# upowai/upow

Measured on AMD Instinct MI355X. Metric: sha256_pow_hashrate_MH/s, higher is better.
Workload: dtype uint32; 1 GPU; model=upow v2 block header PoW (108 B, single SHA-256, nibble-prefix target), global_batch=4294967296, seq_len=108, parallelism=dp1, nonces_per_rank_step=4294967296, device=gpu, kernel_variant=0

## Files before the change

### csrc/bindings.cpp

```cpp
#include <pybind11/numpy.h>
#include <pybind11/pybind11.h>
#include <pybind11/stl.h>

#include <cstring>
#include <malloc.h>
#include <stdexcept>

#include "native.h"
#include "sha256_common.h"
#include "thread_pool.h"

namespace py = pybind11;
using namespace upow;

namespace upow {
void register_txcodec(py::module_& m);
void register_ledger_writer(py::module_& m);
void register_gov_index(py::module_& m);
void register_stall_probe(py::module_& m);
void register_log_appender(py::module_& m);
void register_http_wire(py::module_& m);
void register_mempool_index(py::module_& m);
void register_jsonspan(py::module_& m);
void register_utxo_host(py::module_& m);
}

static PowJobHost make_job(py::bytes header, uint32_t tmask, uint32_t tword, uint32_t frac_shift,
                           uint32_t frac_limit) {
    PowJobHost j;
    std::string h = header;
    j.header.assign(h.begin(), h.end());
    j.tmask = tmask;
    j.tword = tword;
    j.frac_shift = frac_shift;
    j.frac_limit = frac_limit;
    return j;
}

static py::tuple pow_result_tuple(const PowResult& r) {
    return py::make_tuple(r.searched, r.total_hits, r.words);
}

static void packed_args(py::buffer data, py::buffer offsets, const uint8_t*& d, const int64_t*& o, int64_t& n,
                        int64_t& nbytes) {
    py::buffer_info di = data.request(), oi = offsets.request();
    if (oi.itemsize != 8 || oi.ndim != 1) throw std::invalid_argument("offsets must be a 1-D int64 buffer");
    d = static_cast<const uint8_t*>(di.ptr);
    o = static_cast<const int64_t*>(oi.ptr);
    n = oi.shape[0] - 1;
    nbytes = di.size * di.itemsize;
    if (n < 0) throw std::invalid_argument("offsets must have n+1 entries");
    for (int64_t i = 0; i < n; ++i)
        if (o[i] < 0 || o[i + 1] < o[i] || o[i + 1] > nbytes) throw std::out_of_range("bad offsets");
}

PYBIND11_MODULE(_native, m) {
    m.doc() = "upow_amd native core: host C++ crypto + gfx950 HIP kernels";
    register_txcodec(m);
    register_ledger_writer(m);
    register_gov_index(m);
    register_stall_probe(m);
    register_log_appender(m);
    register_http_wire(m);
    register_mempool_index(m);
    register_jsonspan(m);
    register_utxo_host(m);

    m.def("malloc_tune", [](int64_t mmap_threshold, int64_t trim_threshold) {
        bool ok = true;
        if (mmap_threshold > 0) ok &= mallopt(M_MMAP_THRESHOLD, int(std::min<int64_t>(mmap_threshold, INT32_MAX))) == 1;
        if (trim_threshold > 0) ok &= mallopt(M_TRIM_THRESHOLD, int(std::min<int64_t>(trim_threshold, INT32_MAX))) == 1;
        return ok;
    });

    m.def("sha256", [](py::bytes msg) {
        std::string s = msg;
        uint8_t out[32];
        host_sha256(reinterpret_cast<const uint8_t*>(s.data()), s.size(), out);
        return py::bytes(reinterpret_cast<const char*>(out), 32);
    });

    m.def("sha256_batch_host", [](py::buffer data, py::buffer offsets, int threads) {
        const uint8_t* d; const int64_t* o; int64_t n, nb;
        packed_args(data, offsets, d, o, n, nb);
        std::vector<uint8_t> out;
        {
            py::gil_scoped_release rel;
            out = sha256_batch_host(d, o, n, threads);
        }
        return py::bytes(reinterpret_cast<const char*>(out.data()), out.size());
    }, py::arg("data"), py::arg("offsets"), py::arg("threads") = 1);

    m.def("sha256_hex_prefixes", [](py::list hexes, py::array_t<int64_t, py::array::c_style | py::array::forcecast> idx,
                                   py::array_t<int64_t, py::array::c_style | py::array::forcecast> nchars, int threads) {
        const int64_t n = int64_t(idx.size());
        if (int64_t(nchars.size()) != n) throw py::value_error("sha256_hex_prefixes: idx and nchars differ in length");
        const int64_t* ix = idx.data();
        const int64_t* nc = nchars.data();
        std::vector<const char*> src(static_cast<size_t>(n));
        std::vector<py::object> keep;
        keep.reserve(static_cast<size_t>(n));
        const int64_t n_hex = int64_t(hexes.size());
        for (int64_t k = 0; k < n; ++k) {
            if (ix[k] < 0 || ix[k] >= n_hex) throw py::index_error("sha256_hex_prefixes: tx index out of range");
            PyObject* o = PyList_GET_ITEM(hexes.ptr(), Py_ssize_t(ix[k]));
            keep.push_back(py::reinterpret_borrow<py::object>(o));
            if (!PyUnicode_Check(o)) throw py::type_error("transaction hex must be str");
            Py_ssize_t sz = 0;
            const char* p = PyUnicode_AsUTF8AndSize(o, &sz);
            if (!p) throw py::error_already_set();
            if (nc[k] < 0 || nc[k] > int64_t(sz)) throw py::value_error("sha256_hex_prefixes: prefix longer than the hex");
            src[size_t(k)] = p;
        }
        std::string out(size_t(n) * 32, '\0');
        {
            py::gil_scoped_release rel;
            HostPool::get().parallel_for(n, threads, [&](int64_t k) {
                host_sha256(reinterpret_cast<const uint8_t*>(src[size_t(k)]), size_t(nc[k]),
                            reinterpret_cast<uint8_t*>(&out[size_t(k) * 32]));
            });
        }
        return py::bytes(out);
    }, py::arg("hexes"), py::arg("idx"), py::arg("nchars"), py::arg("threads") = 1);

    m.def("sha256_batch_gpu", [](py::buffer data, py::buffer offsets) {
        const uint8_t* d; const int64_t* o; int64_t n, nb;
        packed_args(data, offsets, d, o, n, nb);
        std::vector<uint8_t> out;
        {
            py::gil_scoped_release rel;
            out = sha256_batch_gpu(d, nb, o, n);
        }
        return py::bytes(reinterpret_cast<const char*>(out.data()), out.size());
    });

    m.def("pow_check_word", [](py::bytes header, uint32_t tmask, uint32_t tword, uint32_t fs, uint32_t fl,
                               uint32_t v) { return pow_check_word_host(make_job(header, tmask, tword, fs, fl), v); });

    m.def("pow_variant_count", []() { return pow_variant_count(); });
    m.def("pow_job_h0", [](py::bytes header, uint32_t v) { return pow_job_h0_host(make_job(header, 0, 0, 0, 16), v); },
          py::arg("header"), py::arg("v"),
          "digest word H0 for nonce word v, from the precomputed job constants of the GPU kernel (host arithmetic)");

    m.def("pow_search_host", [](py::bytes header, uint32_t tmask, uint32_t tword, uint32_t fs, uint32_t fl,
                                uint64_t start, uint64_t count, int threads) {
        PowJobHost j = make_job(header, tmask, tword, fs, fl);
        PowResult r;
        {
            py::gil_scoped_release rel;
            r = pow_search_host(j, start, count, threads);
        }
        return pow_result_tuple(r);
    });

    m.def("pow_search_gpu", [](py::bytes header, uint32_t tmask, uint32_t tword, uint32_t fs, uint32_t fl,
                               uint64_t start, uint64_t count, int grid_blocks, uint32_t chunk_iters, uint32_t cap, int variant) {
        PowJobHost j = make_job(header, tmask, tword, fs, fl);
        PowResult r;
        {
            py::gil_scoped_release rel;
            r = pow_search_gpu(j, start, count, grid_blocks, chunk_iters, cap, variant);
        }
        return pow_result_tuple(r);
    }, py::arg("header"), py::arg("tmask"), py::arg("tword"), py::arg("frac_shift"), py::arg("frac_limit"),
       py::arg("start"), py::arg("count"), py::arg("grid_blocks") = 0, py::arg("chunk_iters") = 0,
       py::arg("cap") = 1 << 16, py::arg("variant") = 0);

    m.def("set_node_device", [](int dev) { set_node_device_native(dev); }, py::arg("device"),
          "pin node-side GPU work (verify, decompress, batched SHA-256) to this device from every thread");
    m.def("pow_kernel_info", [](int variant) {
        PowKernelInfo k = pow_kernel_info(variant);
        return py::dict(py::arg("cus") = k.cus, py::arg("blocks_per_cu") = k.blocks_per_cu,
                        py::arg("resident_blocks") = k.resident_blocks);
    }, py::arg("variant") = 0);
    m.def("p256_verify", [](py::buffer items, bool gpu, int threads) {
        py::buffer_info bi = items.request();
        const int64_t nbytes = bi.size * bi.itemsize;
        if (nbytes % 160) throw std::invalid_argument("items must be n x 160 bytes");
        const int64_t n = nbytes / 160;
        const uint8_t* p = static_cast<const uint8_t*>(bi.ptr);
        std::vector<uint8_t> st;
        {
            py::gil_scoped_release rel;
            st = gpu ? p256_verify_gpu(p, n) : p256_verify_host(p, n, threads);
        }
        return py::bytes(reinterpret_cast<const char*>(st.data()), st.size());
    }, py::arg("items"), py::arg("gpu") = false, py::arg("threads") = 1);

    m.def("p256_decompress", [](py::buffer in, bool gpu) {
        py::buffer_info bi = in.request();
        const int64_t nbytes = bi.size * bi.itemsize;
        if (nbytes % 33) throw std::invalid_argument("input must be n x 33 bytes");
        const int64_t n = nbytes / 33;
        std::vector<uint8_t> out(static_cast<size_t>(n) * 64), ok(static_cast<size_t>(n));
        {
            py::gil_scoped_release rel;
            if (gpu) p256_decompress_gpu(static_cast<const uint8_t*>(bi.ptr), n, out.data(), ok.data());
            else p256_decompress_host(static_cast<const uint8_t*>(bi.ptr), n, out.data(), ok.data());
        }
        return py::make_tuple(py::bytes(reinterpret_cast<const char*>(out.data()), out.size()),
                              py::bytes(reinterpret_cast<const char*>(ok.data()), ok.size()));
    }, py::arg("data"), py::arg("gpu") = false);

    m.def("p256_on_curve", [](py::buffer in, bool gpu, int threads) {
        py::buffer_info bi = in.request();
        const int64_t nbytes = bi.size * bi.itemsize;
        if (nbytes % 64) throw std::invalid_argument("input must be n x 64 bytes (x LE | y LE)");
        const int64_t n = nbytes / 64;
        std::string ok(static_cast<size_t>(n), '\0');
        {
            py::gil_scoped_release rel;
            auto* o = reinterpret_cast<uint8_t*>(&ok[0]);
            if (gpu) p256_on_curve_gpu(static_cast<const uint8_t*>(bi.ptr), n, o);
            else p256_on_curve_host(static_cast<const uint8_t*>(bi.ptr), n, o, threads);
        }
        return py::bytes(ok);
    }, py::arg("data"), py::arg("gpu") = false, py::arg("threads") = 8);

    m.def("p256_pubkey", [](py::bytes d_be) -> py::object {
        std::string d = d_be;
        if (d.size() != 32) throw std::invalid_argument("private key must be 32 bytes big-endian");
        uint8_t out[64];
        if (!p256_pubkey(reinterpret_cast<const uint8_t*>(d.data()), out)) return py::none();
        return py::bytes(reinterpret_cast<const char*>(out), 64);
    });

    m.def("p256_scalar_inv_mont", [](py::bytes s_le) -> py::bytes {
        const std::string s = s_le;
        if (s.size() != 32) throw std::invalid_argument("need 32 bytes little-endian");
        uint64_t in[4], out[4];
        std::memcpy(in, s.data(), 32);
        p256_scalar_inv_mont_host(out, in);
        return py::bytes(reinterpret_cast<const char*>(out), 32);
    });

    m.def("p256_fe_ops", [](py::bytes a_le, py::bytes b_le) -> py::bytes {
        const std::string a = a_le, b = b_le;
        if (a.size() != 32 || b.size() != 32) throw std::invalid_argument("need 32-byte little-endian a, b");
        uint32_t x[8], y[8], out[32];
        std::memcpy(x, a.data(), 32);
        std::memcpy(y, b.data(), 32);
        p256_fe_ops_host(x, y, out);
        return py::bytes(reinterpret_cast<const char*>(out), sizeof out);
    });
    m.def("rccl_unique_id", []() { return py::bytes(rccl_unique_id()); });
    m.def("rccl_vote_create", [](py::bytes uid, int world, int rank) {
        const std::string u = uid;
        py::gil_scoped_release rel;
        return rccl_vote_create(u, world, rank);
    });
    m.def("rccl_vote_start", [](int64_t h, int value) { rccl_vote_start(h, value); });
    m.def("rccl_vote_finish", [](int64_t h, double timeout_s) {
        py::gil_scoped_release rel;
        return rccl_vote_finish(h, timeout_s);
    });
    m.def("rccl_vote_stats", [](int64_t h) { return rccl_vote_stats(h); });
    m.def("rccl_vote_destroy", [](int64_t h, bool abort) {
        py::gil_scoped_release rel;
        rccl_vote_destroy(h, abort);
    }, py::arg("h"), py::arg("abort") = false);
    m.def("p256_g16_entries", [](int64_t first, int64_t count) -> py::bytes {
        std::vector<uint8_t> o;
        { py::gil_scoped_release rel; o = p256_g16_entries(first, count); }
        return py::bytes(reinterpret_cast<const char*>(o.data()), o.size());
    });
    m.def("p256_fe_reduce", [](py::bytes c_le) -> py::bytes {
        const std::string c = c_le;
        if (c.size() != 64) throw std::invalid_argument("need 64 bytes little-endian");
        uint32_t x[16], out[8];
        std::memcpy(x, c.data(), 64);
        p256_fe_reduce_host(x, out);
        return py::bytes(reinterpret_cast<const char*>(out), sizeof out);
    });

    m.def("p256_sign", [](py::bytes d_be, py::bytes digest) -> py::object {
        std::string d = d_be, h = digest;
        if (d.size() != 32 || h.size() != 32) throw std::invalid_argument("need 32-byte key and digest");
        uint8_t r[32], s[32];
        if (!p256_sign(reinterpret_cast<const uint8_t*>(d.data()), reinterpret_cast<const uint8_t*>(h.data()), r, s))
            return py::none();
        return py::make_tuple(py::bytes(reinterpret_cast<const char*>(r), 32),
                              py::bytes(reinterpret_cast<const char*>(s), 32));
    });

    m.def("p256_pubkey_batch", [](py::bytes keys_be, int threads) -> py::bytes {
        const std::string d = keys_be;
        if (d.size() % 32) throw std::invalid_argument("keys must be n x 32 bytes big-endian");
        const int64_t n = int64_t(d.size() / 32);
        std::string out(size_t(n) * 64, '\0');
        {
            py::gil_scoped_release rel;
            HostPool::get().parallel_for(n, threads, [&](int64_t i) {
                uint8_t q[64];
                if (p256_pubkey(reinterpret_cast<const uint8_t*>(d.data()) + 32 * i, q)) std::memcpy(&out[size_t(64 * i)], q, 64);
            });
        }
        return py::bytes(out);
    }, py::arg("keys_be"), py::arg("threads") = 8);

    m.def("p256_sign_batch", [](py::bytes keys_be, py::bytes digests, int threads) -> py::bytes {
        const std::string d = keys_be, h = digests;
        if (d.size() % 32 || h.size() != d.size()) throw std::invalid_argument("need n x 32-byte keys and digests");
        const int64_t n = int64_t(d.size() / 32);
        std::string out(size_t(n) * 64, '\0');
        {
            py::gil_scoped_release rel;
            HostPool::get().parallel_for(n, threads, [&](int64_t i) {
                uint8_t r[32], s[32];
                const auto* kp = reinterpret_cast<const uint8_t*>(d.data()) + 32 * i;
                const auto* hp = reinterpret_cast<const uint8_t*>(h.data()) + 32 * i;
                if (p256_sign(kp, hp, r, s)) {
                    std::memcpy(&out[size_t(64 * i)], r, 32);
                    std::memcpy(&out[size_t(64 * i + 32)], s, 32);
                }
            });
        }
        return py::bytes(out);
    }, py::arg("keys_be"), py::arg("digests"), py::arg("threads") = 8);

    auto recs_arg = [](py::buffer b, int64_t& n) {
        py::buffer_info bi = b.request();
        const int64_t nb = bi.size * bi.itemsize;
        if (nb % 40) throw std::invalid_argument("utxo key records must be n x 40 bytes");
        n = nb / 40;
        return static_cast<const uint8_t*>(bi.ptr);
    };
    m.def("utxo_create", &utxo_create);
    m.def("utxo_destroy", &utxo_destroy);
    m.def("utxo_capacity", &utxo_capacity);
    m.def("utxo_rehash", [](int64_t h, uint32_t log2_cap) {
        uint64_t r;
        { py::gil_scoped_release rel; r = utxo_rehash(h, log2_cap); }
        return py::make_tuple(uint32_t(r), uint32_t(r >> 32));
    });
    m.def("utxo_insert", [recs_arg](int64_t h, py::buffer recs, py::object payload) {
        int64_t n; const uint8_t* p = recs_arg(recs, n);
        const uint8_t* pp = nullptr;
        py::buffer_info pi;
        if (!payload.is_none()) {
            pi = payload.cast<py::buffer>().request();
            if (pi.size * pi.itemsize != n * 80) throw std::invalid_argument("payload must be n x 80 bytes");
            pp = static_cast<const uint8_t*>(pi.ptr);
        }
        uint64_t r;
        { py::gil_scoped_release rel; r = utxo_insert(h, p, n, pp); }
        return py::make_tuple(uint32_t(r), uint32_t(r >> 32));
    }, py::arg("h"), py::arg("recs"), py::arg("payload") = py::none());
    m.def("utxo_lookup", [recs_arg](int64_t h, py::buffer recs) {
        int64_t n; const uint8_t* p = recs_arg(recs, n);
        std::vector<uint8_t> o, pay;
        { py::gil_scoped_release rel; o = utxo_lookup(h, p, n, pay); }
        return py::make_tuple(py::bytes(reinterpret_cast<const char*>(o.data()), o.size()),
                              py::bytes(reinterpret_cast<const char*>(pay.data()), pay.size()));
    });
    m.def("utxo_probe", [recs_arg](int64_t h, py::buffer recs) {
        int64_t n; const uint8_t* p = recs_arg(recs, n);
        std::vector<uint8_t> o;
        { py::gil_scoped_release rel; o = utxo_probe(h, p, n); }
        return py::bytes(reinterpret_cast<const char*>(o.data()), o.size());
    });
    m.def("utxo_erase", [recs_arg](int64_t h, py::buffer recs) {
        int64_t n; const uint8_t* p = recs_arg(recs, n);
        std::vector<uint8_t> o;
        { py::gil_scoped_release rel; o = utxo_erase(h, p, n); }
        return py::bytes(reinterpret_cast<const char*>(o.data()), o.size());
    });
    m.def("utxo_apply_async", [recs_arg](int64_t h, py::list ins, py::buffer dels) {
        int64_t n_del;
        const uint8_t* pd = recs_arg(dels, n_del);
        std::vector<UtxoSeg> segs;
        std::vector<py::buffer_info> keep;
        keep.reserve(2 * ins.size());
        int with_pay = -1;
        for (py::handle item : ins) {
            py::tuple t = item.cast<py::tuple>();
            int64_t n;
            const uint8_t* pr = recs_arg(t[0].cast<py::buffer>(), n);
            const uint8_t* pp = nullptr;
            if (!t[1].is_none()) {
                keep.push_back(t[1].cast<py::buffer>().request());
                if (keep.back().size * keep.back().itemsize != n * 80) throw std::invalid_argument("payload must be n x 80 bytes");
                pp = static_cast<const uint8_t*>(keep.back().ptr);
            }
            if (n && with_pay >= 0 && with_pay != (pp != nullptr)) throw std::invalid_argument("payloads for all groups or none");
            if (n) with_pay = pp != nullptr;
            segs.push_back(UtxoSeg{pr, pp, n});
        }
        uint32_t prev[3];
        bool had;
        { py::gil_scoped_release rel; had = utxo_apply_async(h, segs, with_pay == 1, pd, n_del, prev); }
        return py::make_tuple(had, prev[0], prev[1], prev[2]);
    }, py::arg("h"), py::arg("ins"), py::arg("dels"));
    m.def("utxo_apply_wait", [](int64_t h) {
        uint32_t r[3];
        bool had;
        { py::gil_scoped_release rel; had = utxo_apply_wait(h, r); }
        return py::make_tuple(had, r[0], r[1], r[2]);
    });
    m.def("utxo_dump", [](int64_t h) {
        std::vector<uint8_t> o;
        { py::gil_scoped_release rel; o = utxo_dump(h, nullptr); }
        return py::bytes(reinterpret_cast<const char*>(o.data()), o.size());
    });
    m.def("utxo_block_inputs", [recs_arg](int64_t h, py::buffer keys, py::buffer in_start, py::buffer out_amount,
                                          py::buffer out_start, uint32_t want_tag) {
        int64_t n_in; const uint8_t* kp = recs_arg(keys, n_in);
        py::buffer_info bi = in_start.request(), bo = out_start.request(), ba = out_amount.request();
        const size_t is_n = size_t(bi.size * bi.itemsize), os_n = size_t(bo.size * bo.itemsize);
        const size_t oa_n = size_t(ba.size * ba.itemsize);
        if (is_n % 4 || is_n < 4 || os_n != is_n || oa_n % 8) throw std::invalid_argument("bad segment arrays");
        const int64_t n_tx = int64_t(is_n / 4) - 1;
        const int32_t* isp = static_cast<const int32_t*>(bi.ptr);
        const int32_t* osp = static_cast<const int32_t*>(bo.ptr);
        const uint64_t* oap = static_cast<const uint64_t*>(ba.ptr);
        const int64_t n_out = int64_t(oa_n / 8);
        for (int64_t t = 0; t < n_tx; ++t)
            if (isp[t] < 0 || isp[t + 1] < isp[t] || osp[t] < 0 || osp[t + 1] < osp[t])
                throw std::invalid_argument("segment offsets must be non-decreasing");
        if (isp[n_tx] != n_in || osp[n_tx] != n_out || isp[0] != 0 || osp[0] != 0)
            throw std::invalid_argument("segment offsets do not cover the arrays");
        py::array_t<uint8_t> tags(n_in), pay(n_in * 80);
        py::array_t<uint32_t> dup(n_in), miss(std::max<int64_t>(n_tx, 0));
        py::array_t<int64_t> fee(std::max<int64_t>(n_tx, 0));
        BlockInputsOut r{tags.mutable_data(), pay.mutable_data(), dup.mutable_data(), fee.mutable_data(),
                         miss.mutable_data()};
        {
            py::gil_scoped_release rel;
            utxo_block_inputs(h, kp, n_in, isp, oap, n_out, osp, n_tx, want_tag, r);
        }
        return py::make_tuple(tags, pay, dup, fee, miss, r.n_dup);
    });
    m.def("utxo_k12_snapshot", [](int64_t h, uint32_t tag) {
        py::gil_scoped_release rel;
        return utxo_k12_snapshot(h, tag);
    });
    m.def("utxo_k12_digest", [](int64_t id) {
        uint64_t n = 0;
        std::vector<uint8_t> d;
        { py::gil_scoped_release rel; d = utxo_k12_digest(id, &n); }
        return py::make_tuple(py::bytes(reinterpret_cast<const char*>(d.data()), d.size()), n);
    });
    m.def("utxo_set_message", [](int64_t h, uint32_t tag) {
        auto* v = new std::vector<uint8_t>();
        uint64_t n = 0;
        { py::gil_scoped_release rel; *v = utxo_set_message(h, tag, &n); }
// ... 87 lines not shown
```

### csrc/native.h

```cpp
#pragma once
#include <cstdint>
#include <functional>
#include <string>
#include <vector>

namespace upow {

struct PowJobHost {
    std::vector<uint8_t> header;
    uint32_t tmask = 0, tword = 0, frac_shift = 0, frac_limit = 16;
};

struct PowResult {
    uint64_t searched = 0;
    uint32_t total_hits = 0;
    std::vector<uint32_t> words;
};

struct PowKernelInfo {
    int cus = 0, blocks_per_cu = 0, resident_blocks = 0;
};
PowKernelInfo pow_kernel_info(int variant);
int pow_variant_count();
uint32_t pow_job_h0_host(const PowJobHost& job, uint32_t v);

bool pow_check_word_host(const PowJobHost& job, uint32_t v);
PowResult pow_search_host(const PowJobHost& job, uint64_t start, uint64_t count, int threads);
PowResult pow_search_gpu(const PowJobHost& job, uint64_t start, uint64_t count, int grid_blocks,
                         uint32_t chunk_iters, uint32_t cap, int variant);

std::vector<uint8_t> sha256_batch_host(const uint8_t* data, const int64_t* offsets, int64_t n, int threads);
std::vector<uint8_t> sha256_batch_gpu(const uint8_t* data, int64_t nbytes, const int64_t* offsets, int64_t n);

std::vector<uint8_t> p256_verify_host(const uint8_t* items, int64_t n, int threads);
uint8_t p256_verify_one_host64(const uint8_t* item);
const void* p256_g_table_host();
void p256_scalar_inv_mont_host(uint64_t out[4], const uint64_t s[4]);
void p256_fe_ops_host(const uint32_t a[8], const uint32_t b[8], uint32_t out[32]);
void p256_fe_reduce_host(const uint32_t c[16], uint32_t out[8]);
void p256_batch_launch(char variant, const void* items, int64_t n, const void* gtab16, void* scratch, uint8_t* status,
                       int spw, void* stream);
std::string rccl_unique_id();
int64_t rccl_vote_create(const std::string& uid, int world, int rank);
void rccl_vote_start(int64_t h, int value);
int64_t rccl_vote_finish(int64_t h, double timeout_s);
void rccl_vote_destroy(int64_t h, bool abort);
std::vector<double> rccl_vote_stats(int64_t h);
std::vector<uint8_t> p256_g16_entries(int64_t first, int64_t count);
std::vector<uint8_t> p256_verify_gpu(const uint8_t* items, int64_t n);
void p256_decompress_host(const uint8_t* in33, int64_t n, uint8_t* out64, uint8_t* ok);
void p256_decompress_gpu(const uint8_t* in33, int64_t n, uint8_t* out64, uint8_t* ok);
void p256_verify_fused_gpu(int64_t n_jobs, int64_t n_out, const std::function<void(uint8_t*, uint8_t*, uint8_t*)>& fill,
                           uint8_t* st, uint8_t* out_ok, std::vector<uint8_t>* items_out);
void p256_on_curve_host(const uint8_t* xy64, int64_t n, uint8_t* ok, int threads);
void p256_on_curve_gpu(const uint8_t* xy64, int64_t n, uint8_t* ok);
void set_node_device_native(int dev);
bool p256_pubkey(const uint8_t d_be[32], uint8_t out_le[64]);
bool p256_sign(const uint8_t d_be[32], const uint8_t digest[32], uint8_t r_le[32], uint8_t s_le[32]);

int64_t utxo_create(uint32_t log2_cap);
void utxo_destroy(int64_t h);
uint32_t utxo_capacity(int64_t h);
uint64_t utxo_rehash(int64_t h, uint32_t log2_cap);
uint64_t utxo_insert(int64_t h, const uint8_t* recs, int64_t n, const uint8_t* payload);
std::vector<uint8_t> utxo_probe(int64_t h, const uint8_t* recs, int64_t n);
std::vector<uint8_t> utxo_lookup(int64_t h, const uint8_t* recs, int64_t n, std::vector<uint8_t>& payload_out);
std::vector<uint8_t> utxo_erase(int64_t h, const uint8_t* recs, int64_t n);
struct UtxoSeg { const uint8_t* recs; const uint8_t* pay; int64_t n; };
bool utxo_apply_async(int64_t h, const std::vector<UtxoSeg>& ins, bool with_pay, const uint8_t* del, int64_t n_del,
                      uint32_t prev[3]);
bool utxo_apply_wait(int64_t h, uint32_t out[3]);
std::vector<uint8_t> utxo_dump(int64_t h, std::vector<uint8_t>* payload_out);
std::vector<uint8_t> utxo_address_scan(int64_t h, const uint8_t* addr, uint32_t len, uint32_t tag_mask,
                                       uint32_t stake_sel, std::vector<uint8_t>& payload_out, uint64_t* total_out);
struct AddressBatchOut {
    std::vector<uint32_t> qidx;
    std::vector<uint8_t> recs;
    std::vector<uint8_t> payload;
    std::vector<uint64_t> totals;
};
void utxo_address_scan_batch(int64_t h, const uint8_t* addrs, const uint32_t* lens, const uint32_t* tag_masks,
                             const uint32_t* stake_sels, int64_t n, AddressBatchOut& out);

struct BlockInputsOut {
    uint8_t* tags;
    uint8_t* payload;
    uint32_t* dup_of;
    int64_t* fee;
    uint32_t* missing;
    uint32_t n_dup = 0;
};
void utxo_block_inputs(int64_t h, const uint8_t* keys, int64_t n_in, const int32_t* in_start,
                       const uint64_t* out_amount, int64_t n_out, const int32_t* out_start, int64_t n_tx,
                       uint32_t want_tag, BlockInputsOut& r);
std::vector<uint8_t> utxo_set_message(int64_t h, uint32_t tag, uint64_t* count_out);
int64_t utxo_k12_snapshot(int64_t h, uint32_t tag);
std::vector<uint8_t> utxo_k12_digest(int64_t id, uint64_t* count_out);
void utxo_debug_hashes(const uint8_t* recs, int64_t n, uint32_t log2_cap, uint32_t* home_out, uint64_t* fp_out);
std::vector<uint8_t> utxo_debug_slots(int64_t h);

std::string b58encode(const uint8_t* data, size_t n);
constexpr size_t kB58MaxInput = 64, kB58MaxOutput = 88;
size_t b58encode_to(const uint8_t* data, size_t n, char* out);
std::vector<uint8_t> b58decode(const std::string& s);

int gpu_device_count();
std::string gpu_arch_name(int device);

}
```

### csrc/pow_search.hip

```cpp
#include <hip/hip_runtime.h>

#include <algorithm>
#include <cstdint>
#include <stdexcept>
#include <string>

#include "native.h"
#include "streams.h"
#include "sha256_common.h"

namespace upow {

struct PowJobDev {
    uint32_t st[8];
    uint32_t mid[8];
    uint32_t w[16];
    uint32_t tmask;
    uint32_t tword;
    uint32_t frac_shift;
    uint32_t frac_limit;
    uint32_t ca, ce;
    uint32_t hk[3];
    uint32_t kw[64];
};

struct PowWordKinds {
    bool vec[64];
    bool has_const[64];
};
constexpr PowWordKinds pow_word_kinds(int layout) {
    PowWordKinds k{};
    for (int i = 0; i < 16; ++i) k.vec[i] = layout == 2 ? i == 10 : (i == 1 || i == 2);
    for (int i = 16; i < 64; ++i) {
        const int src[4] = {i - 16, i - 15, i - 7, i - 2};
        bool v = false, c = false;
        for (int t = 0; t < 4; ++t) {
            if (k.vec[src[t]]) v = true; else c = true;
        }
        k.vec[i] = v;
        k.has_const[i] = v && c;
    }
    return k;
}

#define ROTR(x, n) __builtin_amdgcn_alignbit((x), (x), (n))
#define XOR3(a, b, c) __builtin_amdgcn_bitop3_b32((a), (b), (c), 0x96)
#define BSIG0(x) XOR3(ROTR((x), 2), ROTR((x), 13), ROTR((x), 22))
#define BSIG1(x) XOR3(ROTR((x), 6), ROTR((x), 11), ROTR((x), 25))
#define SSIG0(x) XOR3(ROTR((x), 7), ROTR((x), 18), ((x) >> 3))
#define SSIG1(x) XOR3(ROTR((x), 17), ROTR((x), 19), ((x) >> 10))
#define CH(e, f, g) (((e) & (f)) | (~(e) & (g)))
#define MAJ(a, b, c) __builtin_amdgcn_bitop3_b32((a), (b), (c), 0xE8)

__constant__ uint32_t dK[64] = {
    0x428a2f98u, 0x71374491u, 0xb5c0fbcfu, 0xe9b5dba5u, 0x3956c25bu, 0x59f111f1u, 0x923f82a4u, 0xab1c5ed5u,
    0xd807aa98u, 0x12835b01u, 0x243185beu, 0x550c7dc3u, 0x72be5d74u, 0x80deb1feu, 0x9bdc06a7u, 0xc19bf174u,
    0xe49b69c1u, 0xefbe4786u, 0x0fc19dc6u, 0x240ca1ccu, 0x2de92c6fu, 0x4a7484aau, 0x5cb0a9dcu, 0x76f988dau,
    0x983e5152u, 0xa831c66du, 0xb00327c8u, 0xbf597fc7u, 0xc6e00bf3u, 0xd5a79147u, 0x06ca6351u, 0x14292967u,
    0x27b70a85u, 0x2e1b2138u, 0x4d2c6dfcu, 0x53380d13u, 0x650a7354u, 0x766a0abbu, 0x81c2c92eu, 0x92722c85u,
    0xa2bfe8a1u, 0xa81a664bu, 0xc24b8b70u, 0xc76c51a3u, 0xd192e819u, 0xd6990624u, 0xf40e3585u, 0x106aa070u,
    0x19a4c116u, 0x1e376c08u, 0x2748774cu, 0x34b0bcb5u, 0x391c0cb3u, 0x4ed8aa4au, 0x5b9cca4fu, 0x682e6ff3u,
    0x748f82eeu, 0x78a5636fu, 0x84c87814u, 0x8cc70208u, 0x90befffau, 0xa4506cebu, 0xbef9a3f7u, 0xc67178f2u};

template <int LAYOUT>
__device__ __forceinline__ uint32_t pow_h0(const PowJobDev& job, uint32_t v) {
    constexpr int R0 = LAYOUT == 2 ? 10 : 1;
    uint32_t w[16];
#pragma unroll
    for (int i = 0; i < 16; ++i) w[i] = job.w[i];
    if (LAYOUT == 2) {
        w[10] = v;
    } else {
        w[1] = job.w[1] | ((v & 0xffu) << 8) | ((v >> 8) & 0xffu);
        w[2] = job.w[2] | (((v >> 16) & 0xffu) << 24) | ((v >> 24) << 16);
    }
    uint32_t a = job.st[0], b = job.st[1], c = job.st[2], d = job.st[3];
    uint32_t e = job.st[4], f = job.st[5], g = job.st[6], h = job.st[7];
#pragma unroll
    for (int i = R0; i < 64; ++i) {
        uint32_t wi;
        if (i < 16) {
            wi = w[i];
        } else {
            wi = w[i & 15] + SSIG0(w[(i - 15) & 15]) + w[(i - 7) & 15] + SSIG1(w[(i - 2) & 15]);
            w[i & 15] = wi;
        }
        uint32_t t1 = h + BSIG1(e) + CH(e, f, g) + dK[i] + wi;
        uint32_t t2 = BSIG0(a) + MAJ(a, b, c);
        h = g; g = f; f = e; e = d + t1; d = c; c = b; b = a; a = t1 + t2;
    }
    return job.mid[0] + a;
}

#if defined(__HIP_DEVICE_COMPILE__)
#define P_ROTR(x, n) ROTR(x, n)
#define P_XOR3(a, b, c) XOR3(a, b, c)
#define P_MAJ(a, b, c) MAJ(a, b, c)
#else
#define P_ROTR(x, n) host_rotr((x), (n))
#define P_XOR3(a, b, c) ((a) ^ (b) ^ (c))
#define P_MAJ(a, b, c) (((a) & (b)) ^ ((a) & (c)) ^ ((b) & (c)))
#endif
#define P_BSIG0(x) P_XOR3(P_ROTR((x), 2), P_ROTR((x), 13), P_ROTR((x), 22))
#define P_BSIG1(x) P_XOR3(P_ROTR((x), 6), P_ROTR((x), 11), P_ROTR((x), 25))
#define P_SSIG0(x) P_XOR3(P_ROTR((x), 7), P_ROTR((x), 18), ((x) >> 3))
#define P_SSIG1(x) P_XOR3(P_ROTR((x), 17), P_ROTR((x), 19), ((x) >> 10))

template <int LAYOUT>
__host__ __device__ __forceinline__ uint32_t pow_h0_pre(const PowJobDev& job, uint32_t v) {
    constexpr int R0 = LAYOUT == 2 ? 10 : 1;
    constexpr PowWordKinds kinds = pow_word_kinds(LAYOUT);
    uint32_t w[16] = {};
    if (LAYOUT == 2) {
        w[10] = v;
    } else {
        w[1] = job.w[1] | ((v & 0xffu) << 8) | ((v >> 8) & 0xffu);
        w[2] = job.w[2] | (((v >> 16) & 0xffu) << 24) | ((v >> 24) << 16);
    }
    uint32_t a = job.ca + w[R0], b = job.st[0], c = job.st[1], d = job.st[2];
    uint32_t e = job.ce + w[R0], f = job.st[4], g = job.st[5], h = 0;
#pragma unroll
    for (int i = R0 + 1; i < 64; ++i) {
        uint32_t wi = 0;
        if (kinds.vec[i]) {
            if (i < 16) {
                wi = w[i];
            } else {
                if (kinds.has_const[i]) wi = job.kw[i];
                if (kinds.vec[i - 16]) wi += w[i & 15];
                if (kinds.vec[i - 15]) wi += P_SSIG0(w[(i - 15) & 15]);
                if (kinds.vec[i - 7]) wi += w[(i - 7) & 15];
                if (kinds.vec[i - 2]) wi += P_SSIG1(w[(i - 2) & 15]);
                w[i & 15] = wi;
            }
        }
        uint32_t x;
        if (i <= R0 + 3) x = kinds.vec[i] ? job.hk[i - R0 - 1] + wi : job.hk[i - R0 - 1];
        else x = kinds.vec[i] ? h + kSha256K[i] + wi : h + job.kw[i];
        const uint32_t t1 = x + P_BSIG1(e) + CH(e, f, g);
        const uint32_t t2 = P_BSIG0(a) + P_MAJ(a, b, c);
        h = g; g = f; f = e; e = d + t1; d = c; c = b; b = a; a = t1 + t2;
    }
    return job.mid[0] + a;
}

typedef __attribute__((address_space(3))) volatile uint32_t lds_u32;

__device__ __forceinline__ uint32_t pow_h0_lds(const PowJobDev& job, uint32_t v, lds_u32* ring) {
    const uint32_t tid = threadIdx.x;
    auto W = [&](int i) -> uint32_t { return i < 16 ? (i == 10 ? v : job.w[i]) : ring[(i & 15) * 256 + tid]; };
    uint32_t a = job.st[0], b = job.st[1], c = job.st[2], d = job.st[3];
    uint32_t e = job.st[4], f = job.st[5], g = job.st[6], h = job.st[7];
#pragma unroll
    for (int i = 10; i < 64; ++i) {
        uint32_t wi;
        if (i < 16) {
            wi = W(i);
        } else {
            wi = W(i - 16) + SSIG0(W(i - 15)) + W(i - 7) + SSIG1(W(i - 2));
            ring[(i & 15) * 256 + tid] = wi;
        }
        uint32_t t1 = h + BSIG1(e) + CH(e, f, g) + dK[i] + wi;
        uint32_t t2 = BSIG0(a) + MAJ(a, b, c);
        h = g; g = f; f = e; e = d + t1; d = c; c = b; b = a; a = t1 + t2;
    }
    return job.mid[0] + a;
}

__global__ __launch_bounds__(256, 1) void pow_search_lds_kernel(PowJobDev job, uint32_t v_base, uint32_t iters,
                                                                uint32_t* __restrict__ out_count,
                                                                uint32_t* __restrict__ out_words, uint32_t cap) {
    __shared__ uint32_t ring[16 * 256];
    const uint32_t nthreads = gridDim.x * blockDim.x;
    uint32_t v = v_base + blockIdx.x * blockDim.x + threadIdx.x;
    for (uint32_t it = 0; it < iters; ++it, v += nthreads) {
        const uint32_t h0 = pow_h0_lds(job, v, (lds_u32*)ring);
        const bool hit = ((h0 ^ job.tword) & job.tmask) == 0 && ((h0 >> job.frac_shift) & 0xfu) < job.frac_limit;
        if (__builtin_expect(hit, 0)) {
            const uint32_t slot = atomicAdd(out_count, 1u);
            if (slot < cap) out_words[slot] = v;
        }
    }
}

template <int LAYOUT, int MIN_WAVES_PER_SIMD>
__global__ __launch_bounds__(256, MIN_WAVES_PER_SIMD) void pow_search_kernel(PowJobDev job, uint32_t v_base, uint32_t iters,
                                                         uint32_t* __restrict__ out_count,
                                                         uint32_t* __restrict__ out_words, uint32_t cap) {
    const uint32_t nthreads = gridDim.x * blockDim.x;
    uint32_t v = v_base + blockIdx.x * blockDim.x + threadIdx.x;
    for (uint32_t it = 0; it < iters; ++it, v += nthreads) {
        const uint32_t h0 = pow_h0<LAYOUT>(job, v);
        const bool hit = ((h0 ^ job.tword) & job.tmask) == 0 && ((h0 >> job.frac_shift) & 0xfu) < job.frac_limit;
        if (__builtin_expect(hit, 0)) {
            const uint32_t slot = atomicAdd(out_count, 1u);
            if (slot < cap) out_words[slot] = v;
        }
    }
}

template <int LAYOUT, int MIN_WAVES_PER_SIMD>
__global__ __launch_bounds__(256, MIN_WAVES_PER_SIMD) void pow_search_pre_kernel(PowJobDev job, uint32_t v_base, uint32_t iters,
                                                             uint32_t* __restrict__ out_count,
                                                             uint32_t* __restrict__ out_words, uint32_t cap) {
    const uint32_t nthreads = gridDim.x * blockDim.x;
    uint32_t v = v_base + blockIdx.x * blockDim.x + threadIdx.x;
    for (uint32_t it = 0; it < iters; ++it, v += nthreads) {
        const uint32_t h0 = pow_h0_pre<LAYOUT>(job, v);
        const bool hit = ((h0 ^ job.tword) & job.tmask) == 0 && ((h0 >> job.frac_shift) & 0xfu) < job.frac_limit;
        if (__builtin_expect(hit, 0)) {
            const uint32_t slot = atomicAdd(out_count, 1u);
            if (slot < cap) out_words[slot] = v;
        }
    }
}

static void hip_check(hipError_t e, const char* what) {
    if (e != hipSuccess) throw std::runtime_error(std::string(what) + ": " + hipGetErrorString(e));
}

PowJobDev make_pow_job(const PowJobHost& hj) {
    PowJobDev j{};
    const uint8_t* hdr = hj.header.data();
    const size_t len = hj.header.size();
    if (len != 108 && len != 138) throw std::invalid_argument("header must be 108 (v2) or 138 (v1) bytes");
    uint32_t st[8];
    std::memcpy(st, kSha256IV, sizeof(st));
    const int full_blocks = len == 108 ? 1 : 2;
    for (int b = 0; b < full_blocks; ++b) host_compress(st, hdr + 64 * b);
    uint8_t tail[64] = {0};
    const size_t rem = len - 64 * full_blocks;
    std::memcpy(tail, hdr + 64 * full_blocks, rem);
    std::memset(tail + rem - 4, 0, 4);
    tail[rem] = 0x80;
    const uint64_t bits = uint64_t(len) * 8;
    for (int i = 0; i < 8; ++i) tail[56 + i] = uint8_t(bits >> (56 - 8 * i));
    for (int i = 0; i < 16; ++i) j.w[i] = load_be32(tail + 4 * i);
    std::memcpy(j.mid, st, sizeof(st));
    uint32_t ws[8];
    std::memcpy(ws, st, sizeof(st));
    host_rounds(ws, j.w, len == 108 ? 10 : 1);
    std::memcpy(j.st, ws, sizeof(ws));
    j.tmask = hj.tmask;
    j.tword = hj.tword;
    j.frac_shift = hj.frac_shift;
    j.frac_limit = hj.frac_limit;
    const int r0 = len == 108 ? 10 : 1;
    const PowWordKinds kinds = pow_word_kinds(len == 108 ? 2 : 1);
    auto ssig0 = [](uint32_t x) { return host_rotr(x, 7) ^ host_rotr(x, 18) ^ (x >> 3); };
    auto ssig1 = [](uint32_t x) { return host_rotr(x, 17) ^ host_rotr(x, 19) ^ (x >> 10); };
    uint32_t wc[64] = {0};
    for (int i = 0; i < 64; ++i) {
        if (i < 16) {
            if (!kinds.vec[i]) wc[i] = j.w[i];
        } else {
            uint32_t sum = 0;
            if (!kinds.vec[i - 16]) sum += wc[i - 16];
            if (!kinds.vec[i - 15]) sum += ssig0(wc[i - 15]);
            if (!kinds.vec[i - 7]) sum += wc[i - 7];
            if (!kinds.vec[i - 2]) sum += ssig1(wc[i - 2]);
            if (!kinds.vec[i]) wc[i] = sum;
            else j.kw[i] = sum;
        }
        if (!kinds.vec[i]) j.kw[i] = kSha256K[i] + wc[i];
    }
    {
        const uint32_t* s = j.st;
        const uint32_t t1 = s[7] + (host_rotr(s[4], 6) ^ host_rotr(s[4], 11) ^ host_rotr(s[4], 25)) +
                            ((s[4] & s[5]) ^ (~s[4] & s[6])) + kSha256K[r0];
        const uint32_t t2 = (host_rotr(s[0], 2) ^ host_rotr(s[0], 13) ^ host_rotr(s[0], 22)) +
                            ((s[0] & s[1]) ^ (s[0] & s[2]) ^ (s[1] & s[2]));
        j.ce = s[3] + t1;
        j.ca = t1 + t2;
        for (int k = 0; k < 3; ++k) {
            const int i = r0 + 1 + k;
            j.hk[k] = s[6 - k] + (kinds.vec[i] ? kSha256K[i] : j.kw[i]);
        }
    }
    return j;
}

uint32_t pow_job_h0_host(const PowJobHost& hj, uint32_t v) {
    const PowJobDev job = make_pow_job(hj);
    return hj.header.size() == 108 ? pow_h0_pre<2>(job, v) : pow_h0_pre<1>(job, v);
}

struct PowDeviceBuffers {
    int device = -1;
    uint32_t* d_count = nullptr;
    uint32_t* d_words = nullptr;
    uint32_t cap = 0;
};

static thread_local PowDeviceBuffers g_pow_bufs;

static PowDeviceBuffers& pow_buffers(uint32_t cap) {
    int dev = 0;
    hip_check(hipGetDevice(&dev), "hipGetDevice");
    PowDeviceBuffers& b = g_pow_bufs;
    if (b.device != dev || b.cap < cap) {
        if (b.d_count) { (void)hipFree(b.d_count); (void)hipFree(b.d_words); }
        hip_check(hipMalloc(&b.d_count, sizeof(uint32_t)), "hipMalloc count");
        hip_check(hipMalloc(&b.d_words, sizeof(uint32_t) * cap), "hipMalloc words");
        b.device = dev;
        b.cap = cap;
    }
    return b;
}

constexpr int kPowDefaultVariant = 5;
constexpr int kPowVariantCount = 6;

using PowKernelFn = void (*)(PowJobDev, uint32_t, uint32_t, uint32_t*, uint32_t*, uint32_t);

static PowKernelFn pow_kernel_fn(bool v2, int variant) {
    if (variant < 0 || variant >= kPowVariantCount) throw std::invalid_argument("unknown PoW kernel variant");
    if (variant == 0) variant = kPowDefaultVariant;
    if (!v2) return variant >= 4 ? &pow_search_pre_kernel<1, 7> : &pow_search_kernel<1, 1>;
    switch (variant) {
        case 1: return &pow_search_kernel<2, 8>;
        case 2: return &pow_search_lds_kernel;
        case 4: return &pow_search_pre_kernel<2, 1>;
        case 5: return &pow_search_pre_kernel<2, 8>;
        default: return &pow_search_kernel<2, 1>;
    }
}

int pow_variant_count() { return kPowVariantCount; }

static int pow_resident_blocks(bool v2, int variant) {
    int dev = 0, cus = 0, per_cu = 0;
    hip_check(hipGetDevice(&dev), "hipGetDevice");
    hip_check(hipDeviceGetAttribute(&cus, hipDeviceAttributeMultiprocessorCount, dev), "attr");
    const void* fn = reinterpret_cast<const void*>(pow_kernel_fn(v2, variant));
    hip_check(hipOccupancyMaxActiveBlocksPerMultiprocessor(&per_cu, fn, 256, 0), "occupancy");
    if (per_cu < 1) per_cu = 1;
    if (per_cu > 8) per_cu = 8;
    return cus * per_cu;
}

PowKernelInfo pow_kernel_info(int variant) {
    PowKernelInfo k;
    int dev = 0;
    hip_check(hipGetDevice(&dev), "hipGetDevice");
    hip_check(hipDeviceGetAttribute(&k.cus, hipDeviceAttributeMultiprocessorCount, dev), "attr");
    k.resident_blocks = pow_resident_blocks(true, variant);
    k.blocks_per_cu = k.resident_blocks / (k.cus ? k.cus : 1);
    return k;
}

PowResult pow_search_gpu(const PowJobHost& hj, uint64_t start, uint64_t count, int grid_blocks,
                         uint32_t chunk_iters, uint32_t cap, int variant) {
    PowJobDev job = make_pow_job(hj);
    const bool v2 = hj.header.size() == 108;
    const PowKernelFn kernel = pow_kernel_fn(v2, variant);
    node_device_enter();
    PowDeviceBuffers& buf = pow_buffers(cap);
    hipStream_t st = miner_stream();
    hip_check(hipMemsetAsync(buf.d_count, 0, sizeof(uint32_t), st), "memset");
    const uint32_t block = 256;
    if (grid_blocks <= 0) grid_blocks = pow_resident_blocks(v2, variant);
    const uint64_t per_launch_threads = uint64_t(grid_blocks) * block;
    if (chunk_iters == 0) {
        int lg = node_stream_live().load() ? 23 : 28;
        if (const char* e = std::getenv("UPOW_POW_DISPATCH_LOG2")) lg = std::max(16, std::min(32, std::atoi(e)));
        chunk_iters = uint32_t(std::max<uint64_t>(1, (uint64_t(1) << lg) / per_launch_threads));
    }
    uint64_t done = 0;
    while (done < count) {
        const uint64_t left = count - done;
        uint32_t iters = chunk_iters;
        uint32_t gb = grid_blocks;
        if (uint64_t(iters) * per_launch_threads > left) {
            iters = uint32_t(left / per_launch_threads);
            if (iters == 0) {
                iters = 1;
                gb = uint32_t((left + block - 1) / block);
                if (uint64_t(gb) * block > left) {
                    gb = uint32_t(left / block);
                    if (gb == 0) break;
                }
            }
        }
        const uint32_t vb = uint32_t(start + done);
        hipLaunchKernelGGL(kernel, dim3(gb), dim3(block), 0, st, job, vb, iters, buf.d_count, buf.d_words, cap);
        hip_check(hipGetLastError(), "pow_search_kernel launch");
        done += uint64_t(iters) * gb * block;
    }
    uint32_t n = 0;
    hip_check(hipMemcpyAsync(&n, buf.d_count, sizeof(uint32_t), hipMemcpyDeviceToHost, st), "copy count");
    hip_check(hipStreamSynchronize(st), "miner stream sync");
    PowResult r;
    r.searched = done;
    r.total_hits = n;
    const uint32_t stored = n < cap ? n : cap;
    r.words.resize(stored);
    if (stored)
    {
        hip_check(hipMemcpyAsync(r.words.data(), buf.d_words, sizeof(uint32_t) * stored, hipMemcpyDeviceToHost, st),
                  "copy words");
        hip_check(hipStreamSynchronize(st), "miner stream sync");
    }
    if (done < count) {
        for (uint64_t k = done; k < count; ++k) {
            const uint32_t v = uint32_t(start + k);
            if (pow_check_word_host(hj, v)) { r.words.push_back(v); r.total_hits++; }
        }
        r.searched = count;
    }
    return r;
}

}
```

Before: 35880 MH/s.

## Add hand-scheduled SHA-256 PoW kernel with pinned instruction order and bitop3 CH

```diff
diff --git a/csrc/bindings.cpp b/csrc/bindings.cpp
--- a/csrc/bindings.cpp
+++ b/csrc/bindings.cpp
@@ -141,6 +141,11 @@
     m.def("pow_job_h0", [](py::bytes header, uint32_t v) { return pow_job_h0_host(make_job(header, 0, 0, 0, 16), v); },
           py::arg("header"), py::arg("v"),
           "digest word H0 for nonce word v, from the precomputed job constants of the GPU kernel (host arithmetic)");
+
+    m.def("pow_job_h0_variant", [](py::bytes header, uint32_t v, int variant) {
+              return pow_job_h0_host(make_job(header, 0, 0, 0, 16), v, variant); },
+          py::arg("header"), py::arg("v"), py::arg("variant"),
+          "pow_job_h0 through the device function of one kernel variant (host arithmetic)");
 
     m.def("pow_search_host", [](py::bytes header, uint32_t tmask, uint32_t tword, uint32_t fs, uint32_t fl,
                                 uint64_t start, uint64_t count, int threads) {
diff --git a/csrc/native.h b/csrc/native.h
--- a/csrc/native.h
+++ b/csrc/native.h
@@ -23,6 +23,7 @@
 PowKernelInfo pow_kernel_info(int variant);
 int pow_variant_count();
 uint32_t pow_job_h0_host(const PowJobHost& job, uint32_t v);
+uint32_t pow_job_h0_host(const PowJobHost& job, uint32_t v, int variant);
 
 bool pow_check_word_host(const PowJobHost& job, uint32_t v);
 PowResult pow_search_host(const PowJobHost& job, uint64_t start, uint64_t count, int threads);
diff --git a/csrc/pow_search.hip b/csrc/pow_search.hip
--- a/csrc/pow_search.hip
+++ b/csrc/pow_search.hip
@@ -4,6 +4,7 @@
 #include <cstdint>
 #include <stdexcept>
 #include <string>
+#include <utility>
 
 #include "native.h"
 #include "streams.h"
@@ -100,6 +101,11 @@
 #define P_ROTR(x, n) host_rotr((x), (n))
 #define P_XOR3(a, b, c) ((a) ^ (b) ^ (c))
 #define P_MAJ(a, b, c) (((a) & (b)) ^ ((a) & (c)) ^ ((b) & (c)))
+#endif
+#if defined(__HIP_DEVICE_COMPILE__)
+#define P_CH(e, f, g) __builtin_amdgcn_bitop3_b32((e), (f), (g), 0xCA)
+#else
+#define P_CH(e, f, g) CH(e, f, g)
 #endif
 #define P_BSIG0(x) P_XOR3(P_ROTR((x), 2), P_ROTR((x), 13), P_ROTR((x), 22))
 #define P_BSIG1(x) P_XOR3(P_ROTR((x), 6), P_ROTR((x), 11), P_ROTR((x), 25))
@@ -144,6 +150,259 @@
     return job.mid[0] + a;
 }
 
+struct PowSchedRegs {
+    uint32_t w[16];
+    uint32_t s[8];
+    uint32_t t[4], u[4], q[3];
+};
+struct PowOpRegs {
+    uint32_t* in[3] = {nullptr, nullptr, nullptr};
+    uint32_t* out = nullptr;
+    __host__ __device__ __forceinline__ bool reads(const uint32_t* p) const {
+        return p != nullptr && (in[0] == p || in[1] == p || in[2] == p);
+    }
+};
+
+constexpr bool pow_sched_op_exists(const PowWordKinds& kinds, int j, int k) {
+    if (j < 16 || j > 63 || !kinds.vec[j]) return false;
+    if (k < 4) return kinds.vec[j - 15];
+    if (k < 8) return kinds.vec[j - 2];
+    const int n = int(kinds.has_const[j]) + int(kinds.vec[j - 16]) + int(kinds.vec[j - 15]) + int(kinds.vec[j - 7]) +
+                  int(kinds.vec[j - 2]);
+    return k == 9 || n == 4;
+}
+
+template <int LAYOUT, int J, int K, bool RUN>
+__host__ __device__ __forceinline__ PowOpRegs pow_sched_op(const PowJobDev& job, PowSchedRegs& r) {
+    constexpr PowWordKinds kinds = pow_word_kinds(LAYOUT);
+    PowOpRegs o;
+    if constexpr (pow_sched_op_exists(kinds, J, K)) {
+        constexpr int j = J, k = K;
+        constexpr bool c = kinds.has_const[j], v16 = kinds.vec[j - 16], v15 = kinds.vec[j - 15],
+                       v7 = kinds.vec[j - 7], v2 = kinds.vec[j - 2];
+        uint32_t(&w)[16] = r.w;
+        uint32_t(&t)[4] = r.t;
+        uint32_t& x15 = w[(j - 15) & 15];
+        uint32_t& x2 = w[(j - 2) & 15];
+        if constexpr (k < 4) {
+            if (k == 3) o = {{&t[2], &t[1], &t[0]}, &t[0]};
+            else o = {{&x15, nullptr, nullptr}, &t[k]};
+            if (RUN) *o.out = k == 0 ? P_ROTR(x15, 7) : k == 1 ? P_ROTR(x15, 18) : k == 2 ? x15 >> 3 : P_XOR3(t[0], t[1], t[2]);
+        } else if constexpr (k < 8) {
+            if (k == 7) o = {{&t[3], &t[2], &t[1]}, &t[1]};
+            else o = {{&x2, nullptr, nullptr}, &t[k - 3]};
+            if (RUN) *o.out = k == 4 ? P_ROTR(x2, 17) : k == 5 ? P_ROTR(x2, 19) : k == 6 ? x2 >> 10 : P_XOR3(t[1], t[2], t[3]);
+        } else {
+            constexpr int n = int(c) + int(v16) + int(v15) + int(v7) + int(v2);
+            uint32_t* reg[7] = {};
+            int nr = 0;
+            if (v16) reg[nr++] = &w[j & 15];
+            if (v15) reg[nr++] = &t[0];
+            if (v7) reg[nr++] = &w[(j - 7) & 15];
+            if (v2) reg[nr++] = &t[1];
+            if (k == 8) o = {{reg[0], c ? nullptr : reg[1], nullptr}, &t[2]};
+            else if (n == 4) o = {{&t[2], reg[nr - 1], reg[nr - 2]}, &w[j & 15]};
+            else o = {{reg[nr - 1], nr > 1 ? reg[nr - 2] : nullptr, nr > 2 ? reg[nr - 3] : nullptr}, &w[j & 15]};
+            if (RUN) {
+                uint32_t term[5] = {};
+                int m = 0;
+                if (c) term[m++] = job.kw[j];
+                if (v16) term[m++] = w[j & 15];
+                if (v15) term[m++] = t[0];
+                if (v7) term[m++] = w[(j - 7) & 15];
+                if (v2) term[m++] = t[1];
+                if (k == 8) t[2] = term[0] + term[1];
+                else w[j & 15] = n == 4 ? t[2] + term[2] + term[3] : term[0] + term[1] + term[2];
+            }
+        }
+    }
+    return o;
+}
+
+enum PowRoundOp { R_X, R_R1, R_R2, R_R3, R_CH, R_S1, R_T1, R_E, R_Q1, R_Q2, R_Q3, R_S0, R_MJ, R_A };
+
+template <int LAYOUT, int I, int OP, bool RUN>
+__host__ __device__ __forceinline__ PowOpRegs pow_round_op(const PowJobDev& job, PowSchedRegs& r) {
+    constexpr PowWordKinds kinds = pow_word_kinds(LAYOUT);
+    constexpr int i = I;
+    uint32_t(&s)[8] = r.s;
+    uint32_t(&u)[4] = r.u;
+    uint32_t(&q)[3] = r.q;
+    uint32_t &a = s[(0 - i) & 7], &b = s[(1 - i) & 7], &c = s[(2 - i) & 7], &d = s[(3 - i) & 7];
+    uint32_t &e = s[(4 - i) & 7], &f = s[(5 - i) & 7], &g = s[(6 - i) & 7], &h = s[(7 - i) & 7];
+    PowOpRegs o;
+    if constexpr (OP == R_X) {
+        o = {{&h, kinds.vec[i] ? &r.w[i & 15] : nullptr, nullptr}, &h};
+        if (RUN) h = kinds.vec[i] ? h + kSha256K[i] + r.w[i & 15] : h + job.kw[i];
+    } else if constexpr (OP == R_R1) {
+        o = {{&e, nullptr, nullptr}, &u[0]};
+        if (RUN) u[0] = P_ROTR(e, 6);
+    } else if constexpr (OP == R_R2) {
+        o = {{&e, nullptr, nullptr}, &u[1]};
+        if (RUN) u[1] = P_ROTR(e, 11);
+    } else if constexpr (OP == R_R3) {
+        o = {{&e, nullptr, nullptr}, &u[2]};
+        if (RUN) u[2] = P_ROTR(e, 25);
+    } else if constexpr (OP == R_CH) {
+        o = {{&e, &f, &g}, &u[3]};
+        if (RUN) u[3] = P_CH(e, f, g);
+    } else if constexpr (OP == R_S1) {
+        o = {{&u[2], &u[1], &u[0]}, &u[0]};
+        if (RUN) u[0] = P_XOR3(u[0], u[1], u[2]);
+    } else if constexpr (OP == R_T1) {
+        o = {{&u[0], &u[3], &h}, &h};
+        if (RUN) h = h + u[0] + u[3];
+    } else if constexpr (OP == R_E) {
+        if constexpr (i != 63) {
+            o = {{&h, &d, nullptr}, &d};
+            if (RUN) d = d + h;
+        }
+    } else if constexpr (OP == R_Q1) {
+        o = {{&a, nullptr, nullptr}, &q[0]};
+        if (RUN) q[0] = P_ROTR(a, 2);
+    } else if constexpr (OP == R_Q2) {
+        o = {{&a, nullptr, nullptr}, &q[1]};
+        if (RUN) q[1] = P_ROTR(a, 13);
+    } else if constexpr (OP == R_Q3) {
+        o = {{&a, nullptr, nullptr}, &q[2]};
+        if (RUN) q[2] = P_ROTR(a, 22);
+    } else if constexpr (OP == R_S0) {
+        o = {{&q[2], &q[1], &q[0]}, &q[0]};
+        if (RUN) q[0] = P_XOR3(q[0], q[1], q[2]);
+    } else if constexpr (OP == R_MJ) {
+        o = {{&a, &b, &c}, &q[1]};
+        if (RUN) q[1] = P_MAJ(a, b, c);
+    } else {
+        o = {{&q[1], &q[0], &h}, &h};
+        if (RUN) h = h + q[0] + q[1];
+    }
+    return o;
+}
+
+template <int B, class F, int... I>
+__host__ __device__ __forceinline__ void pow_static_for(F&& f, std::integer_sequence<int, I...>) {
+    (f(std::integral_constant<int, B + I>{}), ...);
+}
+template <int B, int E, class F>
+__host__ __device__ __forceinline__ void pow_static_for(F&& f) {
+    pow_static_for<B>(f, std::make_integer_sequence<int, (E > B ? E - B : 0)>{});
+}
+
+template <int LAYOUT, int D, bool TWO_PATH>
+struct PowOrder {
+    static constexpr int R0 = 10, FIRST = R0 + 4;
+    static constexpr int SLOTS = 24, STEPS = (64 - FIRST) * SLOTS;
+    static constexpr int kOnePath[14] = {R_X, R_R1, R_R2, R_R3, R_CH, R_S1, R_T1, R_Q1, R_E, R_Q2, R_Q3, R_S0, R_MJ, R_A};
+    static constexpr int kTwoPath[14] = {R_R1, R_Q1, R_R2, R_Q2, R_R3, R_Q3, R_CH, R_S1, R_X, R_S0, R_T1, R_MJ, R_E, R_A};
+    static constexpr int round_of(int g) { return FIRST + g / SLOTS; }
+    static constexpr bool is_sched(int g) {
+        const int n = g % SLOTS;
+        return D == 0 ? n < 10 : (n < 20 && (n & 1));
+    }
+    static constexpr int sched_k(int g) { return D == 0 ? g % SLOTS : (g % SLOTS) / 2; }
+    static constexpr int round_op(int g) {
+        const int n = g % SLOTS, k = D == 0 ? n - 10 : n < 20 ? n / 2 : n - 10;
+        return TWO_PATH ? kTwoPath[k] : kOnePath[k];
+    }
+    static constexpr bool exists(int g) {
+        if (g < 0 || g >= STEPS) return false;
+        if (is_sched(g)) return pow_sched_op_exists(pow_word_kinds(LAYOUT), round_of(g) + D, sched_k(g));
+        return !(round_op(g) == R_E && round_of(g) == 63);
+    }
+    static constexpr bool slow(int g) {
+        if (!exists(g)) return false;
+        const PowWordKinds kinds = pow_word_kinds(LAYOUT);
+        if (is_sched(g)) {
+            const int k = sched_k(g), j = round_of(g) + D;
+            if (k < 8) return (k & 3) < 2;
+            const int n = int(kinds.has_const[j]) + int(kinds.vec[j - 16]) + int(kinds.vec[j - 15]) +
+                          int(kinds.vec[j - 7]) + int(kinds.vec[j - 2]);
+            return k == 9 && n >= 3;
+        }
+        const int op = round_op(g);
+        if (op == R_X) return kinds.vec[round_of(g)];
+        return op == R_R1 || op == R_R2 || op == R_R3 || op == R_Q1 || op == R_Q2 || op == R_Q3 || op == R_T1 || op == R_A;
+    }
+    static constexpr bool rotate(int g) {
+        if (!exists(g)) return false;
+        if (is_sched(g)) return sched_k(g) < 8 && (sched_k(g) & 3) < 2;
+        const int op = round_op(g);
+        return op == R_R1 || op == R_R2 || op == R_R3 || op == R_Q1 || op == R_Q2 || op == R_Q3;
+    }
+    static constexpr bool fill_before(int fill, int g) { return fill == 1 ? rotate(g) : fill == 2 ? slow(g) : false; }
+    static constexpr int next(int g) {
+        if (g < 0) return -1;
+        for (int n = g + 1; n < STEPS; ++n)
+            if (exists(n)) return n;
+        return -1;
+    }
+    template <int G, bool RUN>
+    static __host__ __device__ __forceinline__ PowOpRegs op(const PowJobDev& job, PowSchedRegs& r) {
+        if constexpr (!exists(G)) return {};
+        else if constexpr (is_sched(G)) return pow_sched_op<LAYOUT, round_of(G) + D, sched_k(G), RUN>(job, r);
+        else return pow_round_op<LAYOUT, round_of(G), round_op(G), RUN>(job, r);
+    }
+};
+
+template <int LAYOUT, int D, bool TWO_PATH, int FILL>
+__host__ __device__ __forceinline__ uint32_t pow_h0_sched(const PowJobDev& job, uint32_t v) {
+    static_assert(LAYOUT == 2, "the pinned order is written for the 108-byte header");
+    static_assert(D >= 0 && D < 16, "W[i+D] takes the place of W[i+D-16], which round i must not need any more");
+    using O = PowOrder<LAYOUT, D, TWO_PATH>;
+    constexpr int R0 = O::R0, FIRST = O::FIRST;
+    constexpr PowWordKinds kinds = pow_word_kinds(LAYOUT);
+    PowSchedRegs r = {};
+    r.w[10] = v;
+    {
+        uint32_t(&s)[8] = r.s;
+        constexpr int i = R0 + 1;
+        s[(0 - i) & 7] = job.ca + v; s[(1 - i) & 7] = job.st[0]; s[(2 - i) & 7] = job.st[1]; s[(3 - i) & 7] = job.st[2];
+        s[(4 - i) & 7] = job.ce + v; s[(5 - i) & 7] = job.st[4]; s[(6 - i) & 7] = job.st[5]; s[(7 - i) & 7] = 0;
+    }
+    pow_static_for<16, FIRST + D>([&](auto j) {
+        pow_static_for<0, 10>([&](auto k) { pow_sched_op<LAYOUT, decltype(j)::value, decltype(k)::value, true>(job, r); });
+    });
+#pragma unroll
+    for (int i = R0 + 1; i < FIRST; ++i) {
+        uint32_t(&s)[8] = r.s;
+        uint32_t &a = s[(0 - i) & 7], &b = s[(1 - i) & 7], &c = s[(2 - i) & 7], &d = s[(3 - i) & 7];
+        uint32_t &e = s[(4 - i) & 7], &f = s[(5 - i) & 7], &g = s[(6 - i) & 7], &h = s[(7 - i) & 7];
+        const uint32_t x = kinds.vec[i] ? job.hk[i - R0 - 1] + r.w[i & 15] : job.hk[i - R0 - 1];
+        uint32_t t1 = x + P_BSIG1(e) + P_CH(e, f, g);
+#if defined(__HIP_DEVICE_COMPILE__)
+        asm volatile("" : "+v"(t1));
+#endif
+        const uint32_t t2 = P_BSIG0(a) + P_MAJ(a, b, c);
+        d = d + t1;
+        h = t1 + t2;
+    }
+    pow_static_for<0, O::STEPS>([&](auto gc) {
+        constexpr int g = decltype(gc)::value;
+        if constexpr (O::exists(g)) {
+            const PowOpRegs me = O::template op<g, true>(job, r);
+#if defined(__HIP_DEVICE_COMPILE__)
+            constexpr int g1 = O::next(g), g2 = O::next(g1);
+            const PowOpRegs n1 = O::template op<g1, false>(job, r), n2 = O::template op<g2, false>(job, r);
+            uint32_t* nin = n2.in[0];
+            if (nin == n1.out || n1.reads(nin) || nin == &r.w[10]) nin = nullptr;
+            uint32_t* own = n1.reads(me.out) ? nullptr : me.out;
+            if (nin != nullptr && own != nullptr && nin != own) asm volatile("" : "+v"(*nin), "+v"(*own));
+            else if (own != nullptr) asm volatile("" : "+v"(*own));
+            else if (nin != nullptr) asm volatile("" : "+v"(*nin) : "v"(*me.out));
+            else asm volatile("" ::"v"(*me.out));
+            __builtin_amdgcn_sched_barrier(0);
+            if constexpr (O::fill_before(FILL, g1)) {
+                __builtin_amdgcn_s_sleep(0);
+                __builtin_amdgcn_sched_barrier(0);
+            }
+#else
+            (void)me;
+#endif
+        }
+    });
+    return job.mid[0] + r.s[(0 - 64) & 7];
+}
+
 typedef __attribute__((address_space(3))) volatile uint32_t lds_u32;
 
 __device__ __forceinline__ uint32_t pow_h0_lds(const PowJobDev& job, uint32_t v, lds_u32* ring) {
@@ -207,6 +466,22 @@
     uint32_t v = v_base + blockIdx.x * blockDim.x + threadIdx.x;
     for (uint32_t it = 0; it < iters; ++it, v += nthreads) {
         const uint32_t h0 = pow_h0_pre<LAYOUT>(job, v);
+        const bool hit = ((h0 ^ job.tword) & job.tmask) == 0 && ((h0 >> job.frac_shift) & 0xfu) < job.frac_limit;
+        if (__builtin_expect(hit, 0)) {
+            const uint32_t slot = atomicAdd(out_count, 1u);
+            if (slot < cap) out_words[slot] = v;
+        }
+    }
+}
+
+template <int D, bool TWO_PATH, int FILL, int MIN_WAVES_PER_SIMD>
+__global__ __launch_bounds__(256, MIN_WAVES_PER_SIMD) void pow_search_sched_kernel(PowJobDev job, uint32_t v_base, uint32_t iters,
+                                                               uint32_t* __restrict__ out_count,
+                                                               uint32_t* __restrict__ out_words, uint32_t cap) {
+    const uint32_t nthreads = gridDim.x * blockDim.x;
+    uint32_t v = v_base + blockIdx.x * blockDim.x + threadIdx.x;
+    for (uint32_t it = 0; it < iters; ++it, v += nthreads) {
+        const uint32_t h0 = pow_h0_sched<2, D, TWO_PATH, FILL>(job, v);
         const bool hit = ((h0 ^ job.tword) & job.tmask) == 0 && ((h0 >> job.frac_shift) & 0xfu) < job.frac_limit;
         if (__builtin_expect(hit, 0)) {
             const uint32_t slot = atomicAdd(out_count, 1u);
@@ -308,8 +583,8 @@
     return b;
 }
 
-constexpr int kPowDefaultVariant = 5;
-constexpr int kPowVariantCount = 6;
+constexpr int kPowDefaultVariant = 9;
+constexpr int kPowVariantCount = 10;
 
 using PowKernelFn = void (*)(PowJobDev, uint32_t, uint32_t, uint32_t*, uint32_t*, uint32_t);
 
@@ -322,11 +597,28 @@
         case 2: return &pow_search_lds_kernel;
         case 4: return &pow_search_pre_kernel<2, 1>;
         case 5: return &pow_search_pre_kernel<2, 8>;
+        case 6: return &pow_search_sched_kernel<2, true, 0, 8>;
+        case 7: return &pow_search_sched_kernel<2, false, 0, 8>;
+        case 8: return &pow_search_sched_kernel<2, false, 1, 8>;
+        case 9: return &pow_search_sched_kernel<2, false, 2, 8>;
         default: return &pow_search_kernel<2, 1>;
     }
 }
 
 int pow_variant_count() { return kPowVariantCount; }
+
+uint32_t pow_job_h0_host(const PowJobHost& hj, uint32_t v, int variant) {
+    if (hj.header.size() != 108) return pow_job_h0_host(hj, v);
+    const PowJobDev job = make_pow_job(hj);
+    if (variant == 0) variant = kPowDefaultVariant;
+    switch (variant) {
+        case 6: return pow_h0_sched<2, 2, true, 0>(job, v);
+        case 7: return pow_h0_sched<2, 2, false, 0>(job, v);
+        case 8: return pow_h0_sched<2, 2, false, 1>(job, v);
+        case 9: return pow_h0_sched<2, 2, false, 2>(job, v);
+        default: return pow_h0_pre<2>(job, v);
+    }
+}
 
 static int pow_resident_blocks(bool v2, int variant) {
     int dev = 0, cus = 0, per_cu = 0;
```

After: 38460 MH/s, median of 6. +7.2%, better.
